# phecda-xu/FullyCNNSpeechEnhancement

Measured on AMD Instinct MI355X. Metric: spectrogram frames/sec (CR-CED-16 fwd, 129-bin), higher is better.
Workload: dtype f32; 1 GPU; CR-CED V3 (16-layer, skip connections) forward, batch 256 per GPU, 129x512, fp32 (BASELINE configs[2]); variant=FullyCNNV3, batch_per_gpu=256, frames=512, bins=129, global_batch=256, fused_available=True, parallelism=batch-shard x1, rccl_world_size=1, weights=random-init (glorot, seed 42), library=rced-hip 0.1 gfx950

## Files before the change

fullycnnspeechenhancement_amd/csrc/kernels_fused.hip:

```cpp
#include <hip/hip_runtime.h>

#include <algorithm>
#include <cstdlib>
#include <cstring>
#include <vector>

#include "../../include/rced.h"
#include "kernels_fused_chain.h"
#include "kernels_fused_v3.h"
#include "kernels_frame16.h"
#include "kernels_final_x6.h"
#include "rced_internal.h"

using namespace rced;

inline unsigned short bf16_rne(float f) {
  unsigned u;
  memcpy(&u, &f, 4);
  if ((u & 0x7fffffffu) > 0x7f800000u) return 0x7fc0;
  u += 0x7fffu + ((u >> 16) & 1u);
  return (unsigned short)(u >> 16);
}

inline int env_default(const char* name, int dflt) {
// ... 345 lines not shown
  {
    constexpr int CH = N::kFinalCh;
    using X = x6::FinalX6<CH>;
    const rced_layer_dev& lf = m->layers[N::kLayers];
    std::vector<unsigned short> p(X::kPackShorts, 0);
    auto b2f = [](unsigned short b) { const unsigned u = (unsigned)b << 16; float v; memcpy(&v, &u, 4); return v; };
    for (int S = 0; S < X::kSteps; ++S)
      for (int mt = 0; mt < X::kMT; ++mt)
        for (int lane = 0; lane < 64; ++lane)
          for (int e = 0; e < 8; ++e) {
            const int k = 32 * S + 8 * (lane >> 4) + e, fo = 16 * mt + (lane & 15), fp = k / CH, ci = k % CH, tap = fp - fo + 64;
            const float v = (k < X::kK && fo < 129 && tap >= 0 && tap < 129) ? wq(lf, tap, ci, 0, CH) : 0.f;
            const unsigned short h = bf16_rne(v);
            const float r1 = v - b2f(h);
            const unsigned short mm = bf16_rne(r1);
            const unsigned short l = bf16_rne(r1 - b2f(mm));
            const size_t base = ((size_t)(S * X::kMT + mt) * 3) * 512 + lane * 8 + e;
            p[base] = h;
            p[base + 512] = mm;
            p[base + 1024] = l;
          }
    HIP_TRY(hipMalloc(&f->fin_apack_x6, p.size() * sizeof(unsigned short)));
    HIP_TRY(hipMemcpy(f->fin_apack_x6, p.data(), p.size() * sizeof(unsigned short), hipMemcpyHostToDevice));
  }
  f->scratch_bytes = (size_t)m->num_cus * G::kScratchFloatsPerWg * sizeof(float);
  HIP_TRY(hipMalloc(&f->scratch, f->scratch_bytes));
  HIP_TRY(hipFuncSetAttribute(reinterpret_cast<const void*>(chain::fused_chain_kernel<N>),
                              hipFuncAttributeMaxDynamicSharedMemorySize, G::kLdsBytes));
  using NL = chain::WithTF<N, kLatencyTF>;
  HIP_TRY(hipFuncSetAttribute(reinterpret_cast<const void*>(chain::fused_chain_kernel<NL>),
                              hipFuncAttributeMaxDynamicSharedMemorySize, chain::Geo<NL>::kLdsBytes));
  return RCED_OK;
}

template <class N>
void pack_frame16(const rced_model* m, std::vector<unsigned>* wpack) {
  using G = frame16::Geo<N>;
  wpack->assign(G::kWBytes / 4, 0u);
  for (int l = 0; l < N::kLayers; ++l) {
    const rced_layer_dev& L = m->layers[l];
    const chain::LayerDesc d = N::layer[l];
    const int MT = G::MT(l), OCT = G::oct_in(l);
    unsigned char* pk = reinterpret_cast<unsigned char*>(wpack->data()) + G::packet_off(l);
    unsigned short* d16 = reinterpret_cast<unsigned short*>(pk);
    for (int s = 0; s < G::steps(l); ++s)
      for (int mt = 0; mt < MT; ++mt)
        for (int lane = 0; lane < 64; ++lane)
          for (int e = 0; e < 8; ++e) {
            const int j = 4 * s + (lane >> 4), tap = j / OCT, ch = 8 * (j % OCT) + e, co = 16 * mt + (lane & 15);
            float v = 0.f;
            if (tap < d.taps && co < d.cout) {
              if (l == 0) v = wq(L, e * d.taps + tap, 0, co, 1);
              else if (ch < d.cin) v = wq(L, tap, ch, co, d.cin);
            }
            d16[((size_t)(s * MT + mt) * 64 + lane) * 8 + e] = bf16_rne(v);
          }
    float* sh = reinterpret_cast<float*>(reinterpret_cast<unsigned char*>(wpack->data()) + G::kShiftOff) + 32 * l;
    for (int c = 0; c < d.cout; ++c) sh[c] = L.host_shift[c];
  }
  constexpr int CH = N::kFinalCh, RB = G::kFinRB, CB = G::kFinCB;
  const rced_layer_dev& lf = m->layers[N::kLayers];
  unsigned char* tt = reinterpret_cast<unsigned char*>(wpack->data()) + G::packet_off(N::kLayers);
  auto tapw = [&](int tap, int c) { return bf16_rne((tap >= 0 && tap < 129 && c < CH) ? wq(lf, tap, c, 0, CH) : 0.f); };
  for (int kq = 0; kq < 4; ++kq)
    for (int r = 0; r < G::kTARows; ++r)
      for (int c = 0; c < 8; ++c)
        reinterpret_cast<unsigned short*>(tt + kq * G::kTACopy)[r * 8 + c] = tapw(r + kq - 15, c);
  for (int c = 0; c < RB; ++c)
    for (int k = 0; k < G::kTBRows; ++k)
      for (int j = 0; j < RB; ++j)
        for (int e = 0; e < CB; ++e)
          reinterpret_cast<unsigned short*>(tt + G::kTBOff + c * G::kTBCopy)[(k * RB + j) * CB + e] = tapw(RB * k + c + j - 15, 8 + e);
}
template <class N, int W>
int frame16_prepare(rced_model* m, int* per_cu) {
  using G = frame16::Geo<N, W>;
  const void* k = reinterpret_cast<const void*>(frame16::frame16_kernel<N, W>);
  HIP_TRY(hipFuncSetAttribute(k, hipFuncAttributeMaxDynamicSharedMemorySize, G::kLdsBytes));
  int n = 1;
  if (hipOccupancyMaxActiveBlocksPerMultiprocessor(&n, k, G::kThreads, G::kLdsBytes) != hipSuccess || n < 1) n = 1;
  *per_cu = std::min(n, W == 4 ? 2 : 1);
  return RCED_OK;
}
template <class N>
int frame16_enable(rced_model* m, rced_fused* f) {
  using G = frame16::Geo<N>;
  if (f->wpack16) return RCED_OK;
  std::vector<unsigned> wpack;
  pack_frame16<N>(m, &wpack);
  unsigned* wdev = nullptr;
  HIP_TRY(hipMalloc(&wdev, wpack.size() * sizeof(unsigned)));
  if (hipMemcpy(wdev, wpack.data(), wpack.size() * sizeof(unsigned), hipMemcpyHostToDevice) != hipSuccess) {
    (void)hipFree(wdev);
    return rced_fail(RCED_ERR_HIP, "hipMemcpy(bf16 packets)");
  }
  if (int rc = frame16_prepare<N, 4>(m, &f->bf16_wgs_per_cu)) { (void)hipFree(wdev); return rc; }
  int one = 1;
  if (int rc = frame16_prepare<N, 8>(m, &one)) { (void)hipFree(wdev); return rc; }
  static_assert(G::kScratchBytesPerWave == frame16::Geo<N, 8>::kScratchBytesPerWave, "one scratch serves both forms");
  if (!f->scratch16 && hipMalloc(&f->scratch16, (size_t)8 * m->num_cus * G::kScratchBytesPerWave) != hipSuccess) {
    (void)hipFree(wdev);
    return rced_fail(RCED_ERR_HIP, "hipMalloc(bf16 skip scratch)");
  }
  f->wpack16 = wdev;
  return RCED_OK;
}
template <class N, int W>
int frame16_launch(rced_model* m, rced_fused* f, const float* x, float* y, int Nb, int T, hipStream_t st) {
  using G = frame16::Geo<N, W>;
  frame16::Params P;
  P.x = x;
  P.y = y;
  P.fin_bias = f->fin_bias;
  P.wpack = f->wpack16;
  P.scratch = f->scratch16;
  P.N = Nb;
  P.T = T;
  P.tiles_per_utt = (T + W - 1) / W;
  P.total_tiles = Nb * P.tiles_per_utt;
  P.stamps = nullptr;
#if RCED_F16_STAMPS
  if (!f->stamps && hipMalloc(&f->stamps, 216 * sizeof(unsigned long long)) != hipSuccess) f->stamps = nullptr;
  P.stamps = f->stamps;
#endif
  const int wgs = (W == 4 ? f->bf16_wgs_per_cu : 1) * m->num_cus;
  const int grid = std::min(P.total_tiles, f->grid_limit > 0 ? std::min(f->grid_limit, wgs) : wgs);
  m->prof_begin(RCED_K_FUSED, st);
  hipLaunchKernelGGL((frame16::frame16_kernel<N, W>), dim3(grid), dim3(G::kThreads), G::kLdsBytes, st, P);
  m->prof_end(RCED_K_FUSED, st);
  HIP_TRY(hipGetLastError());
  return RCED_OK;
}
template <class N>
int frame16_forward(rced_model* m, rced_fused* f, const float* x, float* y, int Nb, int T, hipStream_t st) {
  const long long frames = (long long)Nb * T;
  const int w = f->bf16_frames ? f->bf16_frames : frames >= 16LL * m->num_cus ? 8 : 4;
  return w == 8 ? frame16_launch<N, 8>(m, f, x, y, Nb, T, st) : frame16_launch<N, 4>(m, f, x, y, Nb, T, st);
}

int upload(float** dev, const std::vector<float>& host) {
  float* p = nullptr;
  HIP_TRY(hipMalloc(&p, host.size() * sizeof(float)));
  const hipError_t e = hipMemcpy(p, host.data(), host.size() * sizeof(float), hipMemcpyHostToDevice);
  if (e != hipSuccess) {
    (void)hipFree(p);
    return rced_fail(RCED_ERR_HIP, "hipMemcpy(weights): %s", hipGetErrorString(e));
  }
  *dev = p;
  return RCED_OK;
}

}

static_assert(v3::MapA::kLdsBytes == 159024 && v3::MapF32::kLdsBytes == 163024, "update DYNAMIC_LDS in tools/summarize_prof.py");
#if RCED_V3_LEGACY_FORMS
static_assert(v3::MapT::kLdsBytes == 163792 && v3::MapX6::kLdsBytes == 162976, "update DYNAMIC_LDS in tools/summarize_prof.py");
#endif
inline bool v3_form_built(int form) { return form == 0 || form == 3 || (RCED_V3_LEGACY_FORMS && (form == 1 || form == 2)); }
template <class M>
int v3_set_lds() {
  const hipError_t e = hipFuncSetAttribute(reinterpret_cast<const void*>(v3::fused_v3_kernel<M>),
                                           hipFuncAttributeMaxDynamicSharedMemorySize, M::kLdsBytes);
  if (e != hipSuccess) return rced_fail(RCED_ERR_HIP, "hipFuncSetAttribute(LDS %d): %s", M::kLdsBytes, hipGetErrorString(e));
  return RCED_OK;
}
int v3_enable_form(rced_model* m, rced_fused* f, int form) {
  if (!v3_form_built(form)) return rced_fail(RCED_ERR_ARG, "v3_l2x6 takes 3 (the product: every layer at fp32 quality on the bf16 matrix pipe) or 0 (every "
                                                         "layer on the fp32 MFMA, the bit-exact comparator), got %d", form);
  float** dev = form == 0 ? &f->wpack : form == 1 ? &f->wpack_x6 : form == 2 ? &f->wpack_t : &f->wpack_a;
  if (*dev) return RCED_OK;
  std::vector<float> wpack;
  pack_v3(m, form, &wpack);
  float* fresh = nullptr;
  int rc = upload(&fresh, wpack);
  if (!rc && form == 3 && !f->fin_tab) {
    std::vector<float> tab;
    pack_v3_fintab(m, &tab);
    rc = upload(&f->fin_tab, tab);
    if (rc && f->fin_tab) {
      (void)hipFree(f->fin_tab);
      f->fin_tab = nullptr;
    }
  }
#if RCED_V3_LEGACY_FORMS
  if (!rc && (form == 1 || form == 2)) rc = form == 1 ? v3_set_lds<v3::MapX6>() : v3_set_lds<v3::MapT>();
#endif
  if (!rc && (form == 0 || form == 3)) rc = form == 0 ? v3_set_lds<v3::MapF32>() : v3_set_lds<v3::MapA>();
  if (rc) {
    if (fresh) (void)hipFree(fresh);
    return rc;
  }
  *dev = fresh;
  return RCED_OK;
}

int fused_create(rced_model* m) {
  m->fused = nullptr;
  rced_fused* f = new rced_fused();
  f->final_x6 = env_default("RCED_FINAL_X6", 1) != 0;
  f->final_lds = env_default("RCED_FINAL_LDS", 1) != 0;
  if (m->variant != RCED_V3) {
    m->fused = f;
    const int rc = m->variant == RCED_V1 ? chain_create<chain::NetV1>(m, f) : chain_create<chain::NetV2>(m, f);
    if (rc) fused_destroy(m);
    return rc;
  }
  std::vector<float> fin;
  pack_v3_final(m, &fin, &f->fin_bias);
  int rc = upload(&f->fin_apack, fin);
  if (!rc) {
    const int form = env_default("RCED_V3_L2X6", 3);
    f->v3_l2x6 = v3_form_built(form) ? form : 3;
    rc = v3_enable_form(m, f, f->v3_l2x6);
  }
  if (!rc) {
    hipError_t e = hipHostMalloc(reinterpret_cast<void**>(&f->err_host), 64, hipHostMallocMapped);
    if (e == hipSuccess) {
      *f->err_host = 0u;
      e = hipHostGetDevicePointer(reinterpret_cast<void**>(&f->err_dev), f->err_host, 0);
    }
    if (e != hipSuccess) rc = rced_fail(RCED_ERR_HIP, "error word (pinned host memory): %s", hipGetErrorString(e));
  }
#if RCED_STAMPS
  if (!rc && hipMalloc(&f->stamps, (64 + 24 + 128) * sizeof(unsigned long long)) != hipSuccess) f->stamps = nullptr;
#endif
  m->fused = f;
  if (rc) {
    fused_destroy(m);
    return rc;
  }
  return RCED_OK;
}

void fused_destroy(rced_model* m) {
  rced_fused* f = m->fused;
  if (!f) return;
  if (f->wpack) (void)hipFree(f->wpack);
  if (f->wpack_x6) (void)hipFree(f->wpack_x6);
  if (f->wpack_t) (void)hipFree(f->wpack_t);
  if (f->wpack_a) (void)hipFree(f->wpack_a);
  if (f->fin_tab) (void)hipFree(f->fin_tab);
  if (f->wpack16) (void)hipFree(f->wpack16);
  if (f->fin_apack_x6) (void)hipFree(f->fin_apack_x6);
  if (f->scratch16) (void)hipFree(f->scratch16);
  if (f->fin_apack) (void)hipFree(f->fin_apack);
  if (f->h) (void)hipFree(f->h);
  if (f->scratch) (void)hipFree(f->scratch);
  if (f->err_host) (void)hipHostFree(f->err_host);
  delete f;
  m->fused = nullptr;
}

int fused_reserve(rced_model* m, int N, int T) {
  rced_fused* f = m->fused;
  if (m->variant == RCED_V3) return RCED_OK;
  const int ch = m->variant == RCED_V1 ? chain::NetV1::kFinalCh : chain::NetV2::kFinalCh;
  const size_t need = (size_t)N * T * v3::kF * ch * sizeof(float);
  if (need <= f->h_bytes) return RCED_OK;
  if (f->h) {
    HIP_TRY(hipDeviceSynchronize());
    (void)hipFree(f->h);
    f->h = nullptr;
    f->h_bytes = 0;
  }
  HIP_TRY(hipMalloc(&f->h, need));
  f->h_bytes = need;
  return RCED_OK;
}

int fused_check(rced_model* m) {
  rced_fused* f = m->fused;
  if (!f || !f->err_host) return RCED_OK;
  const unsigned e = *reinterpret_cast<volatile unsigned*>(f->err_host);
  if (e == 0u) return RCED_OK;
  return rced_fail(RCED_ERR_STATE, "fused CR-CED kernel: a wave-to-wave hand-off timed out (code %u); results of that "
                                   "launch are invalid -- destroy and recreate the model", e);
}

int fused_forward(rced_model* m, const float* x, float* y, int N, int T, hipStream_t st) {
  rced_fused* f = m->fused;
  if (int rc = fused_reserve(m, N, T)) return rc;
  if (m->variant == RCED_V1)
    return f->bf16 ? frame16_forward<chain::NetV1>(m, f, x, y, N, T, st)
                   : chain_forward<chain::NetV1>(m, f, x, y, N, T, st);
  if (m->variant == RCED_V2)
    return f->bf16 ? frame16_forward<chain::NetV2>(m, f, x, y, N, T, st)
                   : chain_forward<chain::NetV2>(m, f, x, y, N, T, st);
  if (int rc = fused_check(m)) return rc;
  v3::Params P;
  P.err = f->err_dev;
  P.x = x;
  P.y = y;
  P.wpack = f->v3_l2x6 == 3 ? f->wpack_a : f->v3_l2x6 == 2 ? f->wpack_t : f->v3_l2x6 ? f->wpack_x6 : f->wpack;
  P.fin = f->v3_l2x6 == 3 ? f->fin_tab : f->fin_apack;
  P.fin_bias = f->fin_bias;
  P.N = N;
  P.T = T;
  P.tiles_per_utt = (T + v3::kTF - 1) / v3::kTF;
  P.total_tiles = N * P.tiles_per_utt;
  P.stamps = f->stamps;
  const int cus = f->grid_limit > 0 ? f->grid_limit : m->num_cus;
  const int grid = std::min(P.total_tiles, cus);
  m->prof_begin(RCED_K_FUSED, st);
  if (f->v3_l2x6 == 3) hipLaunchKernelGGL(v3::fused_v3_kernel<v3::MapA>, dim3(grid), dim3(v3::kThreads), v3::MapA::kLdsBytes, st, P);
#if RCED_V3_LEGACY_FORMS
  else if (f->v3_l2x6 == 2) hipLaunchKernelGGL(v3::fused_v3_kernel<v3::MapT>, dim3(grid), dim3(v3::kThreads), v3::MapT::kLdsBytes, st, P);
  else if (f->v3_l2x6 == 1) hipLaunchKernelGGL(v3::fused_v3_kernel<v3::MapX6>, dim3(grid), dim3(v3::kThreads), v3::MapX6::kLdsBytes, st, P);
// ... 110 lines not shown
```

fullycnnspeechenhancement_amd/csrc/kernels_fused_v3.h:

```cpp
#pragma once
#include <hip/hip_runtime.h>

#include <type_traits>

#include "lds_dma.h"

#ifndef RCED_V3_LEGACY_FORMS
#define RCED_V3_LEGACY_FORMS 0
#endif
#ifndef RCED_D1
#define RCED_D1 1
#endif
#ifndef RCED_D2
#define RCED_D2 2
#endif
#ifndef RCED_D2X
#define RCED_D2X 1
#endif
#ifndef RCED_D3
#define RCED_D3 2
#endif
#ifndef RCED_LANE_OPAQUE
#define RCED_LANE_OPAQUE 1
#endif
// ... 56 lines not shown
typedef float f32x4 __attribute__((ext_vector_type(4)));
typedef float f32x2 __attribute__((ext_vector_type(2)));
typedef unsigned u32x2 __attribute__((ext_vector_type(2)));
typedef unsigned u32x4 __attribute__((ext_vector_type(4)));
typedef short s16x8 __attribute__((ext_vector_type(8)));
typedef __bf16 bf16x2 __attribute__((ext_vector_type(2)));
typedef __bf16 bf16x8 __attribute__((ext_vector_type(8)));

constexpr int kF = 129;
constexpr int kTF = 4;
constexpr int kS = 133;
constexpr int kNPX = kTF * kS;
constexpr int kWaves = 8;
constexpr int kThreads = kWaves * 64;

constexpr int kB8S = 10;
constexpr int kB8Pad = 4, kB18Pad = 2, kB30Pad = 4;
constexpr int kB8Rows = kB8Pad + kNPX + 4;
constexpr int kB18Rows = kB18Pad + kNPX;
constexpr int kB30Rows = kB30Pad + kNPX;
constexpr int kWRegion = 37 * 128 + 64 + 32;
constexpr int kX0Rows = kTF + 7;
constexpr int kX0Floats = ((kX0Rows * kS + 24 + 3) / 4) * 4;
constexpr int kHS = 10;
constexpr int kHFrame = 193;
constexpr int kHPix = kTF * kHFrame + 64;
constexpr int kFinU = 144, kFinRun = kFinU / kWaves;
constexpr int kFinA = kFinU * 128;
constexpr int kFin128 = 80 * 8;
constexpr int kFinPack = kFinA + kFin128;

template <int FORM>
struct Map {
  static constexpr bool X6 = FORM != 0;
  static constexpr bool kX6 = X6, kFused = false, kAllX6 = false;
  static constexpr int kB8Off = 0;
  static constexpr int kB18Off = kB8Off + kB8Rows * kB8S;
  static constexpr int kPlaneBytes = kB18Rows * 32;
  static constexpr int kRemRows = kB18Rows + 4;
  static constexpr int kRemHMBytes = 3 * kPlaneBytes;
  static constexpr int kRemLBytes = kRemHMBytes + kRemRows * 8;
  static constexpr int kB18Bytes = X6 ? ((kRemLBytes + kRemRows * 4 + 15) / 16) * 16 : kB18Rows * 18 * 4;
  static constexpr int kB30Off = kB18Off + kB18Bytes / 4;
  static constexpr int kWRegions = X6 ? 1 : 2;
  static constexpr int kWOff = kB30Off + kB30Rows * 30;
  static constexpr int kLdsFloats = kWOff + kWRegions * kWRegion;
  static constexpr int kLdsBytes = kLdsFloats * 4;
  static_assert(kLdsBytes <= 160 * 1024, "LDS budget");
  static_assert((kWOff * 4) % 16 == 0 && (kWRegion * 4) % 16 == 0, "LDS-DMA destinations are 16-byte aligned");
  static_assert((kB18Off * 4) % 16 == 0 && (kB30Off % 2) == 0, "aligned buffers");
  static constexpr int kX0Off = kB30Off + kB30Pad * 30;
  static_assert(kX0Floats <= 60 * 30, "X0 must sit inside rows that layer 2 rewrites");
  static constexpr int kHOff = kB18Off + 1200;
  static_assert(kHOff + kHPix * kHS <= kB30Off && (kHOff % 2) == 0, "H fits inside B18");
  static constexpr int kFin128Off = kB18Off + (2 * kPlaneBytes + (kS + kB18Pad) * 32) / 4;
  static_assert(!X6 || (kFin128Off >= kHOff + kHPix * kHS && (kFin128Off * 4) % 16 == 0 &&
                        (kFin128Off + kFin128) * 4 <= kB18Off * 4 + 2 * kPlaneBytes + (kS + kF + kB18Pad) * 32),
                "bin-128 weights: behind H, 16-byte aligned, inside frame 1's real rows of the l plane");
  static constexpr int kFinScr0 = kB30Off + 4112, kFinScr1 = kB30Off + 8112;
  static_assert(kFinScr0 >= kX0Off + kX0Floats && ((kFinScr0 * 4) % 16) == 0 && ((kFinScr1 * 4) % 16) == 0, "16-byte aligned, clear of X0");
  static_assert(kFinScr0 >= kB30Off + (kB30Pad + kF + 4) * 30 && kFinScr0 + 2048 <= kB30Off + (kB30Pad + kS + kF) * 30, "no gap row");
  static_assert(kFinScr1 >= kB30Off + (kB30Pad + kS + kF + 4) * 30 && kFinScr1 + 2048 <= kB30Off + (kB30Pad + 2 * kS + kF) * 30, "no gap row");
  static constexpr int finscr0(int w) { return 4 * kFinScr0 + w * 1024; }
  static constexpr int kFinScrCt = 4 * (kFinScr1 - kFinScr0);
  static constexpr int kScr2Slots = X6 ? 4 : 2;
  static constexpr int kScratch2Off = kB8Off + kB8Pad * kB8S + 8 * kB8S;
  static constexpr int kFlag2Off = kScratch2Off + kScr2Slots * 256;
  static_assert((kScratch2Off * 4) % 16 == 0, "scratch is read/written with b128");
  static_assert(8 + (kScr2Slots * 257 + kB8S - 1) / kB8S <= kF, "layer-2 scratch stays inside frame 0's real pixels");
  static constexpr int kScratchOff = kB18Off + 180;
  static constexpr int kFlagOff = kScratchOff + 3 * 256;
  static_assert((kScratchOff * 4) % 16 == 0, "scratch is read/written with b128");
  static_assert(X6 ? (kScratchOff - kB18Off) * 4 >= (8 + kB18Pad) * 32 && (kFlagOff + 3 - kB18Off) * 4 <= (kF + kB18Pad) * 32
                   : kScratchOff - kB18Off >= (8 + kB18Pad) * 18 && kFlagOff + 3 - kB18Off <= (kF + kB18Pad) * 18,
                "scratch + flags stay inside frame 0's real pixels");
  static_assert(kFlagOff + 3 <= kHOff, "layer 3's hand-off scratch and the H image do not overlap");
  static constexpr int kT1R = 128 * kB8S * 4, kT1W = X6 ? 128 * 32 : 128 * 18 * 4;
  static constexpr int kT2R = !X6 ? 128 * 18 * 4 : RCED_L2_BOTH ? 128 * 32 : 64 * 32;
  static constexpr int kT2W = X6 && !RCED_L2_BOTH ? 64 * 30 * 4 : 128 * 30 * 4;
  static constexpr int kT3R = 128 * 60 * 4, kT3W = 256 * kB8S * 4;
  static constexpr int kTileB18 = X6 ? 16 * 32 : 16 * 18 * 4;
};
typedef Map<0> MapF32;
#if RCED_V3_LEGACY_FORMS
typedef Map<1> MapX6;
#endif

constexpr int kShiftPerLayer = 32;
constexpr int kW1Main = 9 * 128;
constexpr int kW1Rem = 16 * 128;
constexpr int kW1Data = kW1Main + kW1Rem;
constexpr int kL2Steps = 11, kL3Steps = 37;
constexpr int kL2Chunks = 3;
constexpr int kW2Data = kL2Steps * 2 * 128 + 2 * 64;
constexpr int kW3Data = kL3Steps * 128 + 64;
constexpr int kW1 = kW1Data + kShiftPerLayer;
constexpr int kW2 = kW2Data + kShiftPerLayer;
constexpr int kW3 = kW3Data + kShiftPerLayer;
constexpr int kWBlock = kW1 + kW2 + kW3;
constexpr int kWTotal = 5 * kWBlock;
constexpr int kG1Main = 5 * 256, kG1Rem = 8 * 256;
constexpr int kG1 = kG1Main + kG1Rem + kShiftPerLayer;
constexpr int kG2Data = kL2Chunks * 2 * 3 * 64 * 4;
constexpr int kG2 = kG2Data + kShiftPerLayer;
constexpr int kGBlock = kG1 + kG2 + kW3;
constexpr int kGTotal = 5 * kGBlock;
static_assert(kG1 % 4 == 0 && kG2 % 4 == 0 && kW3 % 4 == 0, "16-byte aligned pieces");
static_assert(kW1 + kFin128 <= kWRegion && (kW1 % 4) == 0, "F32 form: the bin-128 weights fit behind a layer-1 packet in its LDS region");

constexpr int kL3MT = 5;
constexpr int kW3TData = kL3MT * 3 * 256;
constexpr int kW3T = kW3TData + kShiftPerLayer;
constexpr int kTBlock = kG1 + kG2 + kW3T;
constexpr int kG1XMain = 9 * 256, kG1XRem = 12 * 256;
constexpr int kG1X = kG1XMain + kG1XRem + kShiftPerLayer;
constexpr int kTBlockX = kG1X + kG2 + kW3T;
constexpr int kTTotal = RCED_T_L1X6 ? kTBlock + 4 * kTBlockX : 5 * kTBlock;
constexpr int kB8PlaneBytes = kB8Rows * 16;
static_assert(kW3T % 4 == 0 && kG2 + kW3T <= 2 * kWRegion, "layer 3's fused-form packet: 16-byte pieces, inside a weight region");
#if RCED_V3_LEGACY_FORMS
#include "kernels_fused_v3_legacy_map.h"
#endif
constexpr int kHFr = 140;
constexpr int kHRows = kTF * kHFr;
constexpr int kHPlaneBytes = kHRows * 16;
constexpr int kHZeroRow = kHRows - 1;
constexpr int kFinTRows = 160;
constexpr int kFinTPart = kFinTRows * 16;
constexpr int kFinTFloats = 3 * kFinTPart / 4;
constexpr int kATotal = 5 * kTBlockX;
template <>
struct Map<3> {
  static constexpr bool X6 = true, kX6 = true, kFused = true, kAllX6 = true, kL1X6 = true;
  static_assert(RCED_T_L1X6 != 0, "the all-x6 form is built on layer1_x6l");
  static constexpr int kB8Off = 0;
  static constexpr int kB8RegionBytes = 3 * (kHPlaneBytes > kB8PlaneBytes ? kHPlaneBytes : kB8PlaneBytes);
  static constexpr int kB18Off = kB8Off + kB8RegionBytes / 4;
  static constexpr int kHalfBytes = ((kB18Rows * 16 + 255) / 256) * 256;
  static constexpr int kRemOff = 2 * kHalfBytes;
  static constexpr int kRemRows = kB18Rows + 6;
  static constexpr int kPlaneBytes = ((kRemOff + kRemRows * 4 + 15) / 16) * 16;
  static constexpr int kRemHMBytes = 0, kRemLBytes = 0;
  static constexpr int kB18Bytes = 3 * kPlaneBytes;
  static constexpr int kWOff = kB18Off + kB18Bytes / 4;
  static constexpr int kW3TOff = kWOff + kG2;
  static constexpr int kWRegions = 1;
  static constexpr int kB30Off = kWOff;
  static constexpr int kW1Off = kW3TOff + kW3T;
  static constexpr int kFinTOff = kW1Off + kG1X;
  static constexpr int kX0Off = kFinTOff + kFinTFloats;
  static constexpr int kHOff = kB8Off, kFin128Off = kB8Off;
  static constexpr int kEdgeOff = kX0Off + kX0Floats;
  static constexpr int kEdgeFlagOff = kEdgeOff + 4 * 2 * 128;
  static constexpr int kLdsFloats = kEdgeFlagOff + 8;
  static constexpr int kLdsBytes = kLdsFloats * 4;
  static_assert(kLdsBytes <= 160 * 1024, "LDS budget");
  static_assert((kB18Off * 4) % 16 == 0 && (kWOff * 4) % 16 == 0 && (kW3TOff * 4) % 16 == 0 && (kW1Off * 4) % 16 == 0 && (kFinTOff * 4) % 16 == 0 &&
                (kX0Off * 4) % 16 == 0 && (kEdgeOff * 4) % 16 == 0, "aligned buffers");
  static constexpr int finscr(int w, int ct) { return kB18Off * 4 + ct * kPlaneBytes + (w >> 2) * kHalfBytes + (kB18Pad + kS * (w & 3)) * 16; }
  static constexpr int kT1R = 128 * kB8S * 4, kT1W = 128 * 16;
  static constexpr int kT2R = 0, kT2W = 0, kT3R = 0, kT3W = 0;
  static constexpr int kTileB18 = 16 * 16;
};
typedef Map<3> MapA;
static_assert(MapA::finscr(7, 2) % 16 == 0 && MapA::finscr(3, 0) + 1024 <= MapA::kB18Off * 4 + (kB18Pad + kS * 3 + kF) * 16, "partial sums: aligned, inside real rows");



struct Params {
  const float* x;
  float* y;
  const float* wpack;
  const float* fin;
  float fin_bias;
  int N, T;
  int tiles_per_utt;
  int total_tiles;
  unsigned long long* stamps;
  unsigned* err;
};

__device__ __forceinline__ f32x4 mfma(float a, float b, f32x4 c) {
  return __builtin_amdgcn_mfma_f32_16x16x4f32(a, b, c, 0, 0, 0);
}
__device__ __forceinline__ f32x4 mfma32(s16x8 a, s16x8 b, f32x4 c) {
  return __builtin_amdgcn_mfma_f32_16x16x32_bf16(__builtin_bit_cast(bf16x8, a), __builtin_bit_cast(bf16x8, b), c, 0, 0, 0);
}
__device__ __forceinline__ void pin() { __builtin_amdgcn_sched_barrier(0); }

__device__ __forceinline__ int opaque(int v) {
  asm volatile("" : "+v"(v));
  return v;
}

template <int NFLOATS>
__device__ __forceinline__ void packet_dma(const float* __restrict__ src, float* dst, int wave, int lane) {
  lane = opaque(lane);
  constexpr int n4 = NFLOATS / 4;
  constexpr int chunks = (n4 + 63) / 64;
#pragma unroll
  for (int i = 0; i < (chunks + kWaves - 1) / kWaves; ++i) {
    const int c = wave + i * kWaves;
    if (c < chunks) {
      if (c * 64 + lane < n4)
        lds_dma16s(src + c * 256, (unsigned)lane * 16u, dst + c * 256);
    }
  }
}
__device__ __forceinline__ void layer_end_sync() {
  asm volatile("s_waitcnt vmcnt(0)" ::: "memory");
  __builtin_amdgcn_s_waitcnt(0x0F70);
#if defined(RCED_T_EXP) && (RCED_T_EXP & 16384)
  asm volatile("s_waitcnt lgkmcnt(0)" ::: "memory");
#else
  __syncthreads();
#endif
}


__device__ __forceinline__ float relu1(float v) {
  const int b = __builtin_bit_cast(int, v);
  return __builtin_bit_cast(float, b > 0 ? b : 0);
}
__device__ __forceinline__ f32x4 relu4(f32x4 v) {
  return f32x4{relu1(v.x), relu1(v.y), relu1(v.z), relu1(v.w)};
}

__device__ __forceinline__ bool px_valid(int px) {
  const int fr = px / kS;
  return px < kNPX && (px - fr * kS) < kF;
}

__device__ __forceinline__ bool span_has_gap(int p0, int len) {
  const int fr = p0 / kS;
  return p0 + len > kNPX || (p0 - fr * kS) + len > kF;
}

struct XStage {
  float v0, v1, v2;
};
__device__ __forceinline__ float xstage_one(const Params& P, bool live, const float* xu, int t0, int e) {
  const int q = e - 4;
  const int r = q >= 0 ? q / kS : -1;
  const int f = q - r * kS;
  const int tt = t0 + r - 3;
  float v = 0.f;
  if (live && e < kX0Floats && q >= 0 && r < kX0Rows && f < kF && tt >= 0 && tt < P.T) v = xu[(size_t)tt * kF + f];
  return v;
}
__device__ __forceinline__ XStage xstage_load(const Params& P, int tile, int tid) {
  tid = opaque(tid);
  const bool live = tile < P.total_tiles;
  const int utt = live ? tile / P.tiles_per_utt : 0;
  const int t0 = live ? (tile - utt * P.tiles_per_utt) * kTF : 0;
  const float* xu = P.x + (size_t)utt * P.T * kF;
  XStage st;
  st.v0 = xstage_one(P, live, xu, t0, tid);
  st.v1 = xstage_one(P, live, xu, t0, tid + kThreads);
  st.v2 = xstage_one(P, live, xu, t0, tid + 2 * kThreads);
  return st;
}
__device__ __forceinline__ void xstage_store(const XStage& st, float* x0, int tid) {
  x0[tid] = st.v0;
  x0[tid + kThreads] = st.v1;
  if (tid + 2 * kThreads < kX0Floats) x0[tid + 2 * kThreads] = st.v2;
}
static_assert(kX0Floats <= 3 * kThreads, "XStage holds 3 floats per thread");

__device__ __forceinline__ void cbar() { asm volatile("" ::: "memory"); }

template <int I, int N, class F>
__device__ __forceinline__ void static_for(F&& f) {
  if constexpr (I < N) {
    f(std::integral_constant<int, I>{});
    static_for<I + 1, N>(f);
  }
}
template <int V>
using IC = std::integral_constant<int, V>;

typedef __attribute__((address_space(3))) char lds_char;
__device__ __forceinline__ unsigned lds_addr(const void* p) {
  return (unsigned)(size_t)(const __attribute__((address_space(3))) char*)p;
}
template <class T>
__device__ __forceinline__ T lds_ld(unsigned base, int imm) {
  return *reinterpret_cast<const __attribute__((address_space(3))) T*>(reinterpret_cast<const lds_char*>(base) + imm);
}
template <class T>
__device__ __forceinline__ void lds_st(unsigned base, int imm, T v) {
  *reinterpret_cast<__attribute__((address_space(3))) T*>(reinterpret_cast<lds_char*>(base) + imm) = v;
}
__device__ __forceinline__ unsigned lds_peek_a(unsigned addr) {
  return *reinterpret_cast<volatile const __attribute__((address_space(3))) unsigned*>(reinterpret_cast<const lds_char*>(addr));
}
__device__ __forceinline__ void lds_poke_a(unsigned addr, unsigned v) {
  *reinterpret_cast<volatile __attribute__((address_space(3))) unsigned*>(reinterpret_cast<lds_char*>(addr)) = v;
}

struct Lane {
  unsigned a8, a4, kq16;
  unsigned rd0, rd0b, rd0r;
  unsigned rd1, rd1b, wr1;
  unsigned rd1r, wr1r;
  unsigned wr1rl;
  unsigned rd2, rd2b, rd2t, rd2tb, wr2;
  unsigned rd2m, rd2r, rd2rl;
// ... 1170 lines not shown
```

fullycnnspeechenhancement_amd/csrc/kernels_fused_v3_l23.h:

```cpp
#pragma once
#ifndef RCED_T_A2REG
#define RCED_T_A2REG 3
#endif
#ifndef RCED_T_PRIO
#define RCED_T_PRIO 1
#endif
#ifndef RCED_T_A3D
#define RCED_T_A3D 1
#endif
#ifndef RCED_T_SGB
#define RCED_T_SGB 1
#endif
#ifndef RCED_T_L1PF
#define RCED_T_L1PF 1
#endif
#ifndef RCED_T_EXP
#define RCED_T_EXP 0
#endif
#if (RCED_T_EXP != 0 || RCED_X6_EXP != 0) && !defined(RCED_TIMING_ONLY)
#error "RCED_T_EXP / RCED_X6_EXP builds compute wrong results: timing experiments only (tools/mkexp.sh ... -DRCED_TIMING_ONLY -DRCED_T_EXP=...)"
#endif

template <int CTRL>
__device__ __forceinline__ float dpp0(float v) {
  return __builtin_bit_cast(float, __builtin_amdgcn_update_dpp(0, __builtin_bit_cast(int, v), CTRL, 0xf, 0xf, true));
}
template <int S>
__device__ __forceinline__ void tap_add(float p, float& oP, float& oC, float& oN) {
  if constexpr (S == 0) {
    oC += p;
  } else if constexpr (S > 0) {
    oC += dpp0<0x110 + S>(p);
    oN += dpp0<0x100 + 16 - S>(p);
  } else {
    oC += dpp0<0x100 - S>(p);
    oP += dpp0<0x110 + 16 + S>(p);
  }
}
__device__ __forceinline__ void mma2(const s16x8 (&a0)[3], const Parts& b0, f32x4& c0, const s16x8 (&a1)[3], const Parts& b1, f32x4& c1) {
  c0 = mfma32(a0[1], b0.m, c0);
  c1 = mfma32(a1[1], b1.m, c1);
  c0 = mfma32(a0[2], b0.h, c0);
  c1 = mfma32(a1[2], b1.h, c1);
  c0 = mfma32(a0[0], b0.l, c0);
  c1 = mfma32(a1[0], b1.l, c1);
  c0 = mfma32(a0[1], b0.h, c0);
  c1 = mfma32(a1[1], b1.h, c1);
  c0 = mfma32(a0[0], b0.m, c0);
  c1 = mfma32(a1[0], b1.m, c1);
  c0 = mfma32(a0[0], b0.h, c0);
  c1 = mfma32(a1[0], b1.h, c1);
}
template <int NM, int NV, int ND = 0>
__device__ __forceinline__ void interleave() {
#if RCED_T_SGB
#pragma unroll
  for (int i = 0; i < NM; ++i) {
    __builtin_amdgcn_sched_group_barrier(0x008, 1, 0);
    if (ND > 0) __builtin_amdgcn_sched_group_barrier(0x100, ND, 0);
    __builtin_amdgcn_sched_group_barrier(0x002, NV, 0);
  }
#endif
}
template <int J>
__device__ __forceinline__ void shift_add(f32x4 pj, float& p0, float& p1, float& c0, float& c1, float& n0, float& n1) {
  if (RCED_T_EXP & 1) {
    c0 += pj.x;
    c1 += pj.z;
    return;
  }
  tap_add<4 - 2 * J>(pj.x, p0, c0, n0);
  if constexpr (2 * J + 1 < 9) tap_add<3 - 2 * J>(pj.y, p0, c0, n0);
  tap_add<4 - 2 * J>(pj.z, p1, c1, n1);
  if constexpr (2 * J + 1 < 9) tap_add<3 - 2 * J>(pj.w, p1, c1, n1);
}

template <class M, bool LAST, class Sp, class Dma1>
__device__ __forceinline__ void layer23(const Params& P, const Lane& L, unsigned lds0, unsigned wbase, const A2Regs& A, int blk, int wave,
                                        unsigned tag, f32x2 (&sk1)[5], f32x2 (&sk2)[5], Sp sp, Dma1 dma1 DET_ARG) {
  DET_BEGIN();
  const bool right = wave >= 4;
  const int fr = wave & 3;
  const unsigned a2 = wbase + L.scr, a3 = a2 + kG2 * 4;
  const f32x4 sh2[2] = {lds_ld<f32x4>(wbase + L.kq16, kG2Data * 4), lds_ld<f32x4>(wbase + L.kq16, (kG2Data + 16) * 4)};
  const f32x2 sh3 = lds_ld<f32x2>(wbase + (L.kq16 >> 1), (kG2 + kW3TData) * 4);
  const f32x4 zero4 = {0.f, 0.f, 0.f, 0.f};
  const f32x2 zero2 = {0.f, 0.f};
  Parts b2[2];
  s16x8 a2m0[3][3];
  if constexpr (RCED_T_A2REG == 3) {
#pragma unroll
    for (int c = 0; c < 3; ++c)
#pragma unroll
      for (int q = 0; q < 3; ++q) a2m0[c][q] = lds_ld<s16x8>(a2, ((2 * c) * 3 + q) * 1024);
  }
  s16x8 a2r[2][2][3];
  unsigned rdc = L.rd2c;
  f32x4 acc2[2][2];
  u32x4 b3h[2], b3m[2], b3l[2];
  s16x8 a3r[RCED_T_A3D + 1][3];
  f32x4 pj[2][2], p4[2] = {zero4, zero4};
  float w0 = -0.f, w1 = -0.f, x0 = -0.f, x1 = -0.f, y0 = -0.f, y1 = -0.f, z0 = -0.f, z1 = -0.f;
  f32x2 hold = zero2;

  auto ldX = [&](auto tc, auto cc) {
    constexpr int t = decltype(tc)::value, c = decltype(cc)::value;
    if ((RCED_T_EXP & 8) && (c > 0 || t > 1)) return;
    Parts& b = b2[(3 * t + c) & 1];
#pragma unroll
    for (int mt = (RCED_T_A2REG == 3 ? 1 : RCED_T_A2REG); mt < 2; ++mt)
#pragma unroll
      for (int q = 0; q < 3; ++q) a2r[(3 * t + c) & 1][mt][q] = lds_ld<s16x8>(a2, ((2 * c + mt) * 3 + q) * 1024);
    if constexpr (c < 2) {
      constexpr int off = t * M::kTileB18 + (M::kAllX6 ? 32 : 64) * c;
      b.h = lds_ld<s16x8>(L.rd2m, off);
      b.m = lds_ld<s16x8>(L.rd2m, off + M::kPlaneBytes);
      b.l = lds_ld<s16x8>(L.rd2m, off + 2 * M::kPlaneBytes);
    } else {
      u32x4 h, m, l;
#pragma unroll
      for (int i = 0; i < 4; ++i) {
        h[i] = lds_ld<unsigned>(rdc, 4 * i);
        m[i] = lds_ld<unsigned>(rdc, 4 * i + M::kPlaneBytes);
        l[i] = lds_ld<unsigned>(rdc, 4 * i + 2 * M::kPlaneBytes);
      }
      b.h = __builtin_bit_cast(s16x8, h);
      b.m = __builtin_bit_cast(s16x8, m);
      b.l = __builtin_bit_cast(s16x8, l);
      rdc += L.rd2cs;
    }
  };
  auto doX = [&](auto tc, auto cc) {
    constexpr int t = decltype(tc)::value, c = decltype(cc)::value, r = (3 * t + c) & 1, u = t & 1;
    if constexpr (c == 0) {
      acc2[u][0] = sh2[0];
      acc2[u][1] = sh2[1];
    }
    mma2(RCED_T_A2REG == 3 ? a2m0[c] : RCED_T_A2REG >= 1 ? A.a[0][c] : a2r[r][0], b2[r], acc2[u][0], RCED_T_A2REG == 2 ? A.a[1][c] : a2r[r][1], b2[r], acc2[u][1]);
  };
  auto split_piece = [&](auto tc, auto qc) {
    constexpr int t = decltype(tc)::value, q = decltype(qc)::value, u = t & 1, mt = q >> 1;
    float v0 = relu1((q & 1) ? acc2[u][mt].z : acc2[u][mt].x), v1 = relu1((q & 1) ? acc2[u][mt].w : acc2[u][mt].y);
    if constexpr (t == 4) {
      const bool ok = vbit(L, kVN0);
      v0 = ok ? v0 : 0.f;
      v1 = ok ? v1 : 0.f;
    }
    P3 p;
    if (RCED_T_EXP & 4) {
      p.h = __builtin_bit_cast(unsigned, v0);
      p.m = __builtin_bit_cast(unsigned, v1);
      p.l = p.h;
    } else {
      p = split2(v0, v1);
    }
    b3h[u][q] = p.h;
    b3m[u][q] = p.m;
    b3l[u][q] = p.l;
  };
  auto ldY = [&](auto jc, auto parc) {
    constexpr int j = decltype(jc)::value, r = (j + decltype(parc)::value) % (RCED_T_A3D + 1);
    if ((RCED_T_EXP & 2) && j > 1) return;
#pragma unroll
    for (int q = 0; q < 3; ++q) a3r[r][q] = lds_ld<s16x8>(a3, (((RCED_T_EXP & 32) ? 0 : j) * 3 + ((RCED_T_EXP & 64) ? 0 : q)) * 1024);
  };
  auto doY = [&](auto uc, auto jc, auto parc) {
    constexpr int u = decltype(uc)::value, j = decltype(jc)::value, r = (j + decltype(parc)::value) % (RCED_T_A3D + 1);
    Parts b;
    b.h = __builtin_bit_cast(s16x8, b3h[u]);
    b.m = __builtin_bit_cast(s16x8, b3m[u]);
    b.l = __builtin_bit_cast(s16x8, b3l[u]);
    if constexpr (j == kL3MT - 1) p4[u] = l2x_mma(a3r[r], b, zero4);
    else pj[u][j & 1] = l2x_mma(a3r[r], b, zero4);
  };
  auto doYY = [&](auto jc, auto parc) {
    constexpr int j = decltype(jc)::value, r = (j + decltype(parc)::value) % (RCED_T_A3D + 1);
    Parts ba, bb;
    ba.h = __builtin_bit_cast(s16x8, b3h[0]);
    ba.m = __builtin_bit_cast(s16x8, b3m[0]);
    ba.l = __builtin_bit_cast(s16x8, b3l[0]);
    bb.h = __builtin_bit_cast(s16x8, b3h[1]);
    bb.m = __builtin_bit_cast(s16x8, b3m[1]);
    bb.l = __builtin_bit_cast(s16x8, b3l[1]);
    f32x4 ca = zero4, cb = zero4;
    mma2(a3r[r], ba, ca, a3r[r], bb, cb);
    if constexpr (j == kL3MT - 1) {
      p4[0] = ca;
      p4[1] = cb;
    } else {
      pj[0][j & 1] = ca;
      pj[1][j & 1] = cb;
    }
  };
  auto finish = [&](auto tc, float s0, float s1) {
    constexpr int t = decltype(tc)::value;
    f32x2 v = {relu1(s0 + sh3.x), relu1(s1 + sh3.y)};
    if constexpr (LAST) {
      v += sk1[t];
    } else {
      v += blk == 3 ? sk2[t] : zero2;
      sk1[t] = blk == 0 ? v : sk1[t];
      sk2[t] = blk == 1 ? v : sk2[t];
    }
    if constexpr (M::kAllX6 && LAST) {
      const P3 p = split2(v.x, v.y);
      if (t < 4 || vbit(L, kVN0)) {
        lds_st<unsigned>(L.wh0, t * 272, p.h);
        lds_st<unsigned>(L.wh0, t * 272 + kHPlaneBytes, p.m);
        lds_st<unsigned>(L.wh0, t * 272 + 2 * kHPlaneBytes, p.l);
      }
    } else if constexpr (RCED_T_L1X6 && !LAST) {
      const P3 p = split2(v.x, v.y);
      if (t < 4 || vbit(L, kVN0)) {
        lds_st<unsigned>(L.wr3p, t * 256, p.h);
        lds_st<unsigned>(L.wr3p, t * 256 + kB8PlaneBytes, p.m);
        lds_st<unsigned>(L.wr3p, t * 256 + 2 * kB8PlaneBytes, p.l);
      }
    } else {
      if (t < 4 || vbit(L, kVN0)) lds_st<f32x2>(LAST ? L.wh0 : L.wr3, t * (16 * kB8S * 4), v);
    }
  };
  static_assert(kHS == kB8S, "one tile stride for both destinations");
  const unsigned edge = lds0 + 4 * M::kEdgeOff + fr * 1024 + L.a8, eflag = lds0 + 4 * M::kEdgeFlagOff + fr * 8;
  auto publish = [&](int dir, float v0, float v1) {
    lds_st<f32x2>(edge, dir * 512, f32x2{v0, v1});
    cbar();
    if (L.a4 == 0) lds_poke_a(eflag + dir * 4, tag);
  };
  auto fetch = [&](int dir) {
    flag_wait(eflag + dir * 4, tag, P.err, 8u);
    return lds_ld<f32x2>(edge, dir * 512);
  };
  auto tail_pair = [&](auto ac) {
    constexpr int a = decltype(ac)::value;
    shift_add<4>(p4[0], w0, w1, x0, x1, y0, y1);
    shift_add<4>(p4[1], x0, x1, y0, y1, z0, z1);
    if constexpr (a == 0) {
      if (right) {
        publish(1, w0, w1);
        hold = f32x2{x0, x1};
      } else {
        finish(IC<0>{}, x0, x1);
      }
    } else {
      finish(IC<a - 1>{}, w0, w1);
      finish(IC<a>{}, x0, x1);
    }
    w0 = y0;
    w1 = y1;
    x0 = z0;
    x1 = z1;
    y0 = y1 = z0 = z1 = -0.f;
  };
  auto runX = [&](auto tc, auto nc, auto prev_tail) {
    constexpr int t = decltype(tc)::value, next = decltype(nc)::value;
    static_for<0, 3>([&](auto cc) {
      constexpr int c = decltype(cc)::value;
      if constexpr (c < 2) ldX(tc, IC<c + 1>{});
      else if constexpr (next == 0) ldX(IC<t + 1>{}, IC<0>{});
      if constexpr (next == 1 && c + RCED_T_A3D >= 3) ldY(IC<c + RCED_T_A3D - 3>{}, IC<0>{});
      if (RCED_T_SGB < 2) pin();
      doX(tc, cc);
      if constexpr (c == 0) prev_tail();
      if constexpr (t > 0) {
        if constexpr (c == 0) {
          split_piece(IC<t - 1>{}, IC<0>{});
          split_piece(IC<t - 1>{}, IC<1>{});
        } else if constexpr (c == 1) {
          split_piece(IC<t - 1>{}, IC<2>{});
          split_piece(IC<t - 1>{}, IC<3>{});
        }
      }
      interleave<12, (c == 0 ? 5 : 3), (RCED_T_SGB >= 2 ? 2 : 0)>();
      pin();
    });
  };
  auto runY = [&](auto ac, auto pairc, auto nc, auto nxc, auto parc, auto prev_tail) {
    constexpr int a = decltype(ac)::value, next = decltype(nc)::value, u0 = a & 1;
    constexpr bool pair = decltype(pairc)::value != 0;
    static_for<0, kL3MT>([&](auto jc) {
      constexpr int j = decltype(jc)::value;
      constexpr int D = RCED_T_A3D, par = decltype(parc)::value, npar = (kL3MT + par) % (D + 1);
      if constexpr (j + D < kL3MT) ldY(IC<j + D>{}, parc);
      else if constexpr (next == 1) ldY(IC<j + D - kL3MT>{}, IC<npar>{});
      if constexpr (next == 0 && j == kL3MT - 1) ldX(nxc, IC<0>{});
      if (RCED_T_SGB < 2) pin();
      if constexpr (pair) doYY(jc, parc);
      else doY(IC<u0>{}, jc, parc);
      if constexpr (j == 0) {
        prev_tail();
      } else {
        shift_add<j - 1>(pj[u0][(j - 1) & 1], w0, w1, x0, x1, y0, y1);
        if constexpr (pair) shift_add<j - 1>(pj[u0 ^ 1][(j - 1) & 1], x0, x1, y0, y1, z0, z1);
      }
      if constexpr (next == 2) sp(jc);
      interleave<(pair ? 12 : 6), (j == 0 ? 4 : 2), (RCED_T_SGB >= 2 ? 1 : 0)>();
      pin();
    });
  };
  auto none = [] {};
  const IC<0> i0;
  const IC<1> i1;
  const IC<2> i2;
  const IC<3> i3;
  const IC<4> i4;

  if (RCED_T_PRIO && right) __builtin_amdgcn_s_setprio(RCED_T_PRIO);
  ldX(i0, i0);
  pin();
  if (!(RCED_T_EXP & 512)) dma1();
  pin();
  runX(i0, i0, none);
  runX(i1, i0, none);
  runX(i2, i1, none);
  DET(0);
  runY(i0, i1, i0, i3, i0, none);
  DET(1);
  if (!right) {
    runX(i3, i1, [&] { tail_pair(i0); });
    DET(2);
    static_for<0, 4>([&](auto qc) { split_piece(i3, qc); });
    runY(i2, i1, i2, i0, i0, none);
    tail_pair(i2);
    publish(0, x0, x1);
    const f32x2 e = fetch(1);
    finish(i3, w0 + e.x, w1 + e.y);
  } else {
    runX(i3, i0, [&] { tail_pair(i0); });
    runX(i4, i1, none);
    DET(2);
    runY(i2, i1, i1, i0, i0, none);
    static_for<0, 4>([&](auto qc) { split_piece(i4, qc); });
    runY(i4, i0, i2, i0, IC<kL3MT % (RCED_T_A3D + 1)>{}, [&] { tail_pair(i2); });
    shift_add<4>(p4[0], w0, w1, x0, x1, y0, y1);
    finish(i3, w0, w1);
    finish(i4, x0, x1);
    const f32x2 e = fetch(0);
    finish(i0, hold.x + e.x, hold.y + e.y);
    if (RCED_T_PRIO) __builtin_amdgcn_s_setprio(0);
  }
  DET(3);
}


__device__ __forceinline__ Parts b8_load(unsigned rd, int off) {
  Parts b;
  b.h = lds_ld<s16x8>(rd, off);
  if (RCED_T_EXP & 256) {
    b.m = b.l = b.h;
    return b;
  }
  b.m = lds_ld<s16x8>(rd, off + kB8PlaneBytes);
  b.l = lds_ld<s16x8>(rd, off + 2 * kB8PlaneBytes);
  return b;
}

template <class M>
constexpr int a1x_off(int i) {
  if constexpr (M::kAllX6) return M::kW1Off * 4 + i * 1024;
  else return i < 5 ? M::kX0Off * 4 + i * 1024
                    : M::kHOff * 4 + (kHFrame * ((i - 5) / 4) + 64) * kHS * 4 + 8 * (((i - 5) / 4) & 1) + ((i - 5) % 4) * 1024;
}
template <class M>
constexpr int a1x_shift_off() {
  if constexpr (M::kAllX6) return M::kW1Off * 4 + 21 * 1024;
  else return M::kX0Off * 4 + 5 * 1024;
}
#if RCED_V3_LEGACY_FORMS
static_assert(a1x_shift_off<MapT>() + 128 <= (MapT::kX0Off + kX0Floats) * 4 && a1x_off<MapT>(20) + 1024 <= (MapT::kHOff + (kHFrame * 3 + 64 + kF) * kHS) * 4 &&
              a1x_off<MapT>(8) % 16 == 0 && a1x_off<MapT>(9) % 16 == 0 && a1x_off<MapT>(13) % 16 == 0 && a1x_off<MapT>(17) % 16 == 0,
              "layer 1's LDS-resident images: inside the input-row area / the real bins of the H image, 16-byte aligned");
#endif
template <class M>
__device__ __forceinline__ void a1x_dma(const float* src, float* lds, int wave, int lane) {
  lane = opaque(lane);
#pragma unroll
  for (int k = 0; k < 3; ++k) {
    const int ci = wave + 8 * k;
    if (ci < 21) {
      lds_dma16s(src + ci * 256, (unsigned)lane * 16u, lds + a1x_off<M>(ci) / 4);
    } else if (ci == 21) {
      if (lane < 8) lds_dma16s(src + 21 * 256, (unsigned)lane * 16u, lds + a1x_shift_off<M>() / 4);
    }
  }
}
template <class M, int I>
__device__ __forceinline__ s16x8 a1x_ld(unsigned aX, unsigned aH) {
  if constexpr (I < 5 || M::kAllX6) return lds_ld<s16x8>(aX, I * 1024);
  else return lds_ld<s16x8>(aH, a1x_off<M>(I) - M::kHOff * 4);
}
template <class M, class Dma, class Sp>
__device__ __forceinline__ void layer1_x6l(const Lane& L, unsigned lds0, int role, Dma dma, Sp sp DET_ARG) {
  DET_BEGIN();
  constexpr int kTW = M::kT1W, kTR = 128 * 16;
  const unsigned aX = lds0 + (M::kAllX6 ? a1x_off<M>(0) : M::kX0Off * 4) + L.scr, aH = lds0 + M::kHOff * 4 + L.scr;
  const f32x4 sh = lds_ld<f32x4>(lds0 + a1x_shift_off<M>() + L.kq16, 0);
  const f32x2 s2 = lds_ld<f32x2>(lds0 + a1x_shift_off<M>(), 64);
  auto pre = once(dma);
  auto lda = [&](auto pc, s16x8 (&a)[3]) {
    constexpr int g = decltype(pc)::value;
    a[0] = a1x_ld<M, 3 * g>(aX, aH);
    a[1] = a1x_ld<M, 3 * g + 1>(aX, aH);
    a[2] = a1x_ld<M, 3 * g + 2>(aX, aH);
  };
  constexpr bool kPF = M::kAllX6 && RCED_T_L1PF;
  const bool has_single = role < 2 || role == 7, has_rem = role >= 4;
  const unsigned rd_single = L.rd1x + (role == 0 ? 32 : role == 1 ? 30 : 16) * 256;
  Parts nb;
  s16x8 na[3];
  auto prefetch = [&](unsigned rd, int aoff) {
    nb = b8_load(rd, 0);
#pragma unroll
    for (int q = 0; q < 3; ++q) na[q] = lds_ld<s16x8>(aX + aoff, q * 1024);
  };
  {
    Parts b[2][2];
    s16x8 a[3][3];
    f32x4 acc[2][2];
    const bool two = role != 7;
    const bool g1 = tile_has_gap(role + 8), g2 = tile_has_gap(role + 16), g3 = tile_has_gap(role + 24);
    auto ld = [&](auto ic) {
      constexpr int i = decltype(ic)::value, p = i / 3, c = i % 3;
      if constexpr (p == 0) lda(IC<c>{}, a[c]);
      b[i & 1][0] = b8_load(L.rd1x, 2 * p * kTR + 64 * c);
      b[i & 1][1] = b8_load(L.rd1xb, 2 * p * kTR + 64 * c);
    };
    auto slot = [&](auto ic) {
      constexpr int i = decltype(ic)::value, p = i / 3, c = i % 3;
      if constexpr (c == 0) acc[p][0] = acc[p][1] = sh;
      mma2(a[c], b[i & 1][0], acc[p][0], a[c], b[i & 1][1], acc[p][1]);
      if constexpr (p == 0) static_for<0, 3>([&](auto qc) { sp(IC<12 + 3 * i + decltype(qc)::value>{}); });
      if constexpr (p == 1 && c == 0) l1_store<M>(L, acc[0][0], L.wr1, 0, false, kVMain);
      if constexpr (p == 1 && c == 1) l1_store<M>(L, acc[0][1], L.wr1, kTW, g1, kVMain + 1);
      interleave<12, 3>();
    };
    ld(IC<0>{});
    pin();
    if (!(RCED_T_EXP & 512)) pre();
    pin();
    static_for<0, 3>([&](auto ic) {
      constexpr int i = decltype(ic)::value;
      if constexpr (i < 2) ld(IC<i + 1>{});
      else if (two) ld(IC<3>{});
      pin();
      slot(ic);
      pin();
      DETX(i);
    });
    if (two) {
      static_for<3, 6>([&](auto ic) {
        constexpr int i = decltype(ic)::value;
        if constexpr (i < 5) ld(IC<i + 1>{});
        pin();
        slot(ic);
        pin();
        DETX(i);
      });
      if constexpr (kPF) {
        if (has_single) prefetch(rd_single, 0);
        else if (has_rem) prefetch(L.rd1xr, 9 * 1024);
        pin();
      }
      l1_store<M>(L, acc[1][0], L.wr1, 2 * kTW, g2, kVMain + 2);
      l1_store<M>(L, acc[1][1], L.wr1, 3 * kTW, g3, kVMain + 3);
      DETX(6);
    } else {
      if constexpr (kPF) {
        prefetch(rd_single, 0);
        pin();
      }
      l1_store<M>(L, acc[0][0], L.wr1, 0, false, 0);
      l1_store<M>(L, acc[0][1], L.wr1, kTW, false, 0);
    }
  }
  DET(6);
  if (RCED_T_EXP & 8192) return;
  if (role < 2 || role == 7) {
    const int dt = role == 0 ? 32 : role == 1 ? 30 : 16;
    const unsigned rd = L.rd1x + dt * 256;
// ... 82 lines not shown
```

Measured before the change: 22.78 million frames/s.

## Offload layer-2/3 tail tiles to helper waves via LDS flags in all-X6 form

For the all-X6 map, four waves (starting at RCED_T_TAILW) compute the layer-2 tail tile and the layer-3 tail partial products early. They store the split hi/mid/lo results in a new LDS tail region and signal readiness with flags. The right-half waves then take a shorter path and add these precomputed tail contributions, instead of running the extra runX/runY/split work for the i4 tile. This rebalances work across waves, at the cost of about 1.4KB more LDS, new flag waits, and extra early work on the helper waves.

Measured after the change: 23.19 million frames/s (median of 6 runs). 1.8% higher.

```diff
diff --git a/fullycnnspeechenhancement_amd/csrc/kernels_fused.hip b/fullycnnspeechenhancement_amd/csrc/kernels_fused.hip
--- a/fullycnnspeechenhancement_amd/csrc/kernels_fused.hip
+++ b/fullycnnspeechenhancement_amd/csrc/kernels_fused.hip
@@ -521,7 +521,7 @@
 
 }
 
-static_assert(v3::MapA::kLdsBytes == 159024 && v3::MapF32::kLdsBytes == 163024, "update DYNAMIC_LDS in tools/summarize_prof.py");
+static_assert(v3::MapA::kLdsBytes == 160448 && v3::MapF32::kLdsBytes == 163024, "update DYNAMIC_LDS in tools/summarize_prof.py");
 #if RCED_V3_LEGACY_FORMS
 static_assert(v3::MapT::kLdsBytes == 163792 && v3::MapX6::kLdsBytes == 162976, "update DYNAMIC_LDS in tools/summarize_prof.py");
 #endif
diff --git a/fullycnnspeechenhancement_amd/csrc/kernels_fused_v3.h b/fullycnnspeechenhancement_amd/csrc/kernels_fused_v3.h
--- a/fullycnnspeechenhancement_amd/csrc/kernels_fused_v3.h
+++ b/fullycnnspeechenhancement_amd/csrc/kernels_fused_v3.h
@@ -232,7 +232,9 @@
   static constexpr int kHOff = kB8Off, kFin128Off = kB8Off;
   static constexpr int kEdgeOff = kX0Off + kX0Floats;
   static constexpr int kEdgeFlagOff = kEdgeOff + 4 * 2 * 128;
-  static constexpr int kLdsFloats = kEdgeFlagOff + 8;
+  static constexpr int kTailOff = kEdgeFlagOff + 8;
+  static constexpr int kTailFloats = (2 * 3 * 16 * 8 + 4 * 5 * 4 * 8 + 16) / 4;
+  static constexpr int kLdsFloats = kTailOff + kTailFloats;
   static constexpr int kLdsBytes = kLdsFloats * 4;
   static_assert(kLdsBytes <= 160 * 1024, "LDS budget");
   static_assert((kB18Off * 4) % 16 == 0 && (kWOff * 4) % 16 == 0 && (kW3TOff * 4) % 16 == 0 && (kW1Off * 4) % 16 == 0 && (kFinTOff * 4) % 16 == 0 &&
diff --git a/fullycnnspeechenhancement_amd/csrc/kernels_fused_v3_l23.h b/fullycnnspeechenhancement_amd/csrc/kernels_fused_v3_l23.h
--- a/fullycnnspeechenhancement_amd/csrc/kernels_fused_v3_l23.h
+++ b/fullycnnspeechenhancement_amd/csrc/kernels_fused_v3_l23.h
@@ -4,6 +4,9 @@
 #endif
 #ifndef RCED_T_PRIO
 #define RCED_T_PRIO 1
+#endif
+#ifndef RCED_T_TAILW
+#define RCED_T_TAILW 4
 #endif
 #ifndef RCED_T_A3D
 #define RCED_T_A3D 1
@@ -75,6 +78,11 @@
   if constexpr (2 * J + 1 < 9) tap_add<3 - 2 * J>(pj.w, p1, c1, n1);
 }
 
+template <class M>
+constexpr int tail_off() {
+  if constexpr (M::kAllX6) return M::kTailOff;
+  else return 0;
+}
 template <class M, bool LAST, class Sp, class Dma1>
 __device__ __forceinline__ void layer23(const Params& P, const Lane& L, unsigned lds0, unsigned wbase, const A2Regs& A, int blk, int wave,
                                         unsigned tag, f32x2 (&sk1)[5], f32x2 (&sk2)[5], Sp sp, Dma1 dma1 DET_ARG) {
@@ -305,12 +313,87 @@
   const IC<3> i3;
   const IC<4> i4;
 
+  const int tln = (int)(L.a4 >> 2), tn = tln & 15, tkq = tln >> 4, tf = tn & 3;
+  const unsigned tb = lds0 + 4 * tail_off<M>();
+  constexpr int kT3 = 2 * 3 * 16 * 8, kTFlag = kT3 + 4 * 5 * 4 * 8;
+  auto tail2 = [&](auto, int mt) {
+    const unsigned PL = lds0 + 4 * M::kB18Off, px = kS * tf + 64;
+    const unsigned rm = PL + (tkq & 1) * M::kHalfBytes + (px + (tkq >> 1)) * 16;
+    const unsigned rc = tkq < 2 ? rm + 64 + 4 * M::kTileB18 : PL + M::kRemOff + (px + 4 * (tkq & 1)) * 4 + 4 * 64;
+    const unsigned am = a2 + (unsigned)mt * 3072u;
+    f32x4 acc = mt ? sh2[1] : sh2[0];
+    static_for<0, 3>([&](auto cc) {
+      constexpr int c = decltype(cc)::value;
+      Parts b;
+      if constexpr (c < 2) {
+        b.h = lds_ld<s16x8>(rm, 4 * M::kTileB18 + 32 * c);
+        b.m = lds_ld<s16x8>(rm, 4 * M::kTileB18 + 32 * c + M::kPlaneBytes);
+        b.l = lds_ld<s16x8>(rm, 4 * M::kTileB18 + 32 * c + 2 * M::kPlaneBytes);
+      } else {
+        u32x4 h, m, l;
+#pragma unroll
+        for (int i = 0; i < 4; ++i) {
+          h[i] = lds_ld<unsigned>(rc, 4 * i);
+          m[i] = lds_ld<unsigned>(rc, 4 * i + M::kPlaneBytes);
+          l[i] = lds_ld<unsigned>(rc, 4 * i + 2 * M::kPlaneBytes);
+        }
+        b.h = __builtin_bit_cast(s16x8, h);
+        b.m = __builtin_bit_cast(s16x8, m);
+        b.l = __builtin_bit_cast(s16x8, l);
+      }
+      s16x8 a[3];
+#pragma unroll
+      for (int q = 0; q < 3; ++q) a[q] = lds_ld<s16x8>(am, (6 * c + q) * 1024);
+      acc = l2x_mma(a, b, acc);
+    });
+    const P3 p0 = split2(relu1(acc.x), relu1(acc.y)), p1 = split2(relu1(acc.z), relu1(acc.w));
+    const unsigned r = tb + (unsigned)(mt * 3 * 16 + tkq * 4 + tf) * 8u;
+    lds_st<u32x2>(r, 0, u32x2{p0.h, p1.h});
+    lds_st<u32x2>(r, 16 * 8, u32x2{p0.m, p1.m});
+    lds_st<u32x2>(r, 32 * 8, u32x2{p0.l, p1.l});
+    cbar();
+    if (L.a4 == 0) lds_poke_a(tb + kTFlag + 4 * mt, tag);
+  };
+  auto tail3 = [&](auto j0c, auto j1c) {
+    constexpr int j0 = decltype(j0c)::value, j1 = decltype(j1c)::value;
+    flag_wait(tb + kTFlag, tag, P.err, 8u);
+    flag_wait(tb + kTFlag + 4, tag, P.err, 8u);
+    const unsigned r = tb + (unsigned)(tkq * 4 + tf) * 8u;
+    Parts b;
+    const u32x2 h0 = lds_ld<u32x2>(r, 0), m0 = lds_ld<u32x2>(r, 16 * 8), l0 = lds_ld<u32x2>(r, 32 * 8);
+    const u32x2 h1 = lds_ld<u32x2>(r, 48 * 8), m1 = lds_ld<u32x2>(r, 64 * 8), l1 = lds_ld<u32x2>(r, 80 * 8);
+    b.h = __builtin_bit_cast(s16x8, u32x4{h0[0], h0[1], h1[0], h1[1]});
+    b.m = __builtin_bit_cast(s16x8, u32x4{m0[0], m0[1], m1[0], m1[1]});
+    b.l = __builtin_bit_cast(s16x8, u32x4{l0[0], l0[1], l1[0], l1[1]});
+    static_for<j0, j1>([&](auto jc) {
+      constexpr int j = decltype(jc)::value;
+      s16x8 a[3];
+#pragma unroll
+      for (int q = 0; q < 3; ++q) a[q] = lds_ld<s16x8>(a3, (j * 3 + q) * 1024);
+      const f32x4 p = l2x_mma(a, b, zero4);
+      const unsigned o = tb + kT3 + (unsigned)((tf * 5 + 2 * j - 4) * 4 + tkq) * 8u;
+      lds_st<f32x2>(o, 0, f32x2{p.x, p.z});
+      if constexpr (2 * j + 1 < 9) lds_st<f32x2>(o, 32, f32x2{p.y, p.w});
+    });
+    cbar();
+    if (L.a4 == 0) lds_poke_a(tb + kTFlag + 8 + 4 * (j0 == 2 ? 0 : 1), tag);
+  };
+  const bool tail = M::kAllX6 && !(RCED_T_EXP & 1024);
+
   if (RCED_T_PRIO && right) __builtin_amdgcn_s_setprio(RCED_T_PRIO);
+  const int tw = wave - RCED_T_TAILW;
+  if constexpr (M::kAllX6) {
+    if (tail && (tw == 0 || tw == 1)) tail2(i0, tw);
+  }
   ldX(i0, i0);
   pin();
   if (!(RCED_T_EXP & 512)) dma1();
   pin();
   runX(i0, i0, none);
+  if constexpr (M::kAllX6) {
+    if (tail && tw == 2) tail3(i2, i4);
+    else if (tail && tw == 3) tail3(i4, IC<5>{});
+  }
   runX(i1, i0, none);
   runX(i2, i1, none);
   DET(0);
@@ -325,6 +408,30 @@
     publish(0, x0, x1);
     const f32x2 e = fetch(1);
     finish(i3, w0 + e.x, w1 + e.y);
+  } else if (M::kAllX6) {
+    runX(i3, i1, [&] { tail_pair(i0); });
+    DET(2);
+    static_for<0, 4>([&](auto qc) { split_piece(i3, qc); });
+    runY(i2, i1, i2, i0, i0, none);
+    tail_pair(i2);
+    if (tail) {
+      flag_wait(tb + kTFlag + 8, tag, P.err, 8u);
+      flag_wait(tb + kTFlag + 12, tag, P.err, 8u);
+      const int ti = tn >= 12 ? 16 - tn : 0;
+      const f32x2 r = lds_ld<f32x2>(tb + kT3 + (unsigned)((fr * 5 + ti) * 4 + tkq) * 8u, 0);
+      if (tn >= 12) {
+        w0 += r.x;
+        w1 += r.y;
+      } else if (tn == 0) {
+        x0 += r.x;
+        x1 += r.y;
+      }
+    }
+    finish(i3, w0, w1);
+    finish(i4, x0, x1);
+    const f32x2 e = fetch(0);
+    finish(i0, hold.x + e.x, hold.y + e.y);
+    if (RCED_T_PRIO) __builtin_amdgcn_s_setprio(0);
   } else {
     runX(i3, i0, [&] { tail_pair(i0); });
     runX(i4, i1, none);
```
